# mabdullahsoyturk/Torch-Sputnik

Measured on AMD Instinct MI355X. Metric: SpMM effective GFLOP/s (2*nnz*N/t), M=N=K=4096 fp32, density 0.1, higher is better.
Workload: dtype f32

## Files before the change

torch_sputnik_amd/csrc/gen_spmm_flat.py:

```python
#!/usr/bin/env python3
import argparse

_ap = argparse.ArgumentParser()
_ap.add_argument("--mode", default="entry", choices=["entry", "group"])
_ap.add_argument("--layout", default="straight", choices=["straight", "diagonal"])
_ap.add_argument("out", nargs="?")
ARGS = _ap.parse_args()
GROUP = ARGS.mode == "group"

BK = 32
BK_SHIFT = 5
ROW_BYTES = 2048
ROW_SHIFT = 11
WIN_BYTES = 144
NSTRIP = 4
NPIECES = 4
ROWSTEP = 8

V_LANE, V_STAGE, V_PLAN, V_ROWS = "v0", "v1", "v2", "v3"
CUR_OFF, CUR_VAL = 4, 5
NXT_OFF, NXT_VAL, NXT_ROWS = 6, 7, 8
NN_OFF, NN_VAL, NN_ROWS = 10, 11, 12
PAIR = [16, 18, 20, 22]
VALT = [16, 18]
V_ADDR = 20
STRIP = [32, 40, 48, 56]
ACC = 64

S_STREAM, S_VALUES, S_CINFO, S_DENSE = "s[36:37]", "s[38:39]", "s[40:41]", "s[42:43]"
S_PITCH, S_KMAX, S_NCHUNKS, S_ROW0, S_LDS0, S_DEBUG = "s44", "s45", "s46", "s47", "s48", "s49"
S_REM, S_C, S_CIOFF, S_MINE, S_SB, S_NSW = "s50", "s51", "s56", "s57", "s76", "s77"
S_CI = ["s52", "s53", "s54", "s55"]
S_RET, S_BND = "s[58:59]", "s[60:61]"
S_ROWS = [62, 63, 64, 65]
S_IDX = [66, 67, 68, 69]
S_COLS = "s78"
S_T = ["s70", "s71", "s72", "s73", "s74", "s75"]

out = []


def emit(line):
    out.append(line)


def label(name):
    return f".L_{name}_%="


def strip_reads(ring, addr):
    s = STRIP[ring]
    emit(f"ds_read_b128 v[{s}:{s + 3}], v{addr}")
    emit(f"ds_read_b128 v[{s + 4}:{s + 7}], v{addr} offset:1024")


def fmas(src_pair, op_sel, ring):
    s = STRIP[ring]
    for q in range(4):
        emit(f"v_pk_fma_f32 v[{ACC + 2 * q}:{ACC + 2 * q + 1}], v[{src_pair}:{src_pair + 1}], "
             f"v[{s + 2 * q}:{s + 2 * q + 1}], v[{ACC + 2 * q}:{ACC + 2 * q + 1}] {op_sel}")


def entry_fma_stage(ring, lgkm):
    emit(f"s_waitcnt lgkmcnt({lgkm})")
    emit(f"s_set_gpr_idx_on s{S_IDX[ring]}, 0xc")
    fmas(PAIR[ring], "op_sel:[1,0,0] op_sel_hi:[1,1,1]", ring)
    emit("s_set_gpr_idx_off")


def entry_slot(slot):
    ring = slot % NSTRIP
    p = PAIR[ring]
    emit(f"{label(f'E_{slot}')}:")
    emit(f"s_sub_u32 {S_REM}, {S_REM}, 1")
    emit(f"s_cbranch_scc1 {label(f'bnd_{slot}')}")
    emit(f"v_mov_b64_dpp v[{p}:{p + 1}], v[{CUR_OFF}:{CUR_VAL}] row_newbcast:{slot} row_mask:0xf bank_mask:0xf")
    emit(f"s_bfe_u32 s{S_IDX[ring]}, s{S_ROWS[slot // 4]}, {hex(8 * (slot % 4) | (7 << 16))}")
    emit(f"v_add_u32 v{p}, v{p}, {V_LANE}")
    strip_reads(ring, p)
    entry_fma_stage((ring + 1) % NSTRIP, 2 * (NSTRIP - 1))


def group_entry_body(ring, slot):
    t = VALT[slot % 2]
    emit(f"v_mov_b32_dpp v{t}, v{CUR_VAL} row_newbcast:{slot} row_mask:0xf bank_mask:0xf")
    emit(f"s_bfe_u32 s{S_IDX[0]}, s{S_ROWS[slot // 4]}, {hex(8 * (slot % 4) | (7 << 16))}")
    emit(f"s_set_gpr_idx_on s{S_IDX[0]}, 0xc")
    fmas(t, "op_sel:[0,0,0] op_sel_hi:[0,1,1]", ring)
    emit("s_set_gpr_idx_off")


def group_start(ring, slot):
    emit(f"{label(f'N_{ring}_{slot}')}:")
    emit(f"s_sub_u32 {S_REM}, {S_REM}, 1")
    emit(f"s_cbranch_scc1 {label(f'bnd_{slot}')}")
    emit(f"v_mov_b32_dpp v{V_ADDR}, v{CUR_OFF} row_newbcast:{slot} row_mask:0xf bank_mask:0xf")
    emit(f"v_add_u32 v{V_ADDR}, v{V_ADDR}, {V_LANE}")
    strip_reads(ring, V_ADDR)
    emit(f"s_waitcnt lgkmcnt({2 * (NSTRIP - 1)})")


def first_groups():
    for i in range(NSTRIP - 1):
        emit(f"s_bfe_u32 {S_T[0]}, {S_COLS}, {hex(8 * i | (8 << 16))}")
        emit(f"s_lshl_b32 {S_T[0]}, {S_T[0]}, {ROW_SHIFT}")
        emit(f"v_add_u32 v{V_ADDR}, {S_T[0]}, {V_LANE}")
        strip_reads(i, V_ADDR)


def stage_chunk(chunk_sgpr):
    t_row, t_lds, t_r, t_lo, t_hi = S_T[1], S_T[2], S_T[3], S_T[4], S_T[5]
    emit(f"s_lshl_b32 {t_row}, {chunk_sgpr}, {BK_SHIFT}")
    emit(f"s_add_u32 {t_row}, {t_row}, {S_ROW0}")
    emit(f"s_and_b32 {t_lds}, {chunk_sgpr}, 1")
    emit(f"s_lshl_b32 {t_lds}, {t_lds}, 16")
    emit(f"s_add_u32 {t_lds}, {t_lds}, {S_LDS0}")
    for i in range(NPIECES):
        emit(f"s_add_u32 {t_r}, {t_row}, {ROWSTEP * i}")
        emit(f"s_min_u32 {t_r}, {t_r}, {S_KMAX}")
        emit(f"s_mul_hi_u32 {t_hi}, {t_r}, {S_PITCH}")
        emit(f"s_mul_i32 {t_lo}, {t_r}, {S_PITCH}")
        emit(f"s_add_u32 {t_lo}, {t_lo}, s42")
        emit(f"s_addc_u32 {t_hi}, {t_hi}, s43")
        emit(f"s_add_u32 m0, {t_lds}, {hex(ROWSTEP * i * ROW_BYTES)}")
        emit("s_nop 0")
        emit(f"global_load_lds_dwordx4 {V_STAGE}, s[{t_lo[1:]}:{t_hi[1:]}]")


def plan_load(off, rows):
    emit(f"global_load_dwordx2 v[{off}:{off + 1}], {V_PLAN}, {S_STREAM}")
    emit(f"global_load_dword v{rows}, {V_ROWS}, {S_STREAM}")
    emit(f"v_add_u32 {V_PLAN}, {hex(WIN_BYTES)}, {V_PLAN}")
    emit(f"v_add_u32 {V_ROWS}, {hex(WIN_BYTES)}, {V_ROWS}")


def gather(val):
    emit(f"global_load_dword v{val}, v{val}, {S_VALUES}")


def switch_window(tag):
    emit(f"s_cmp_lg_u32 {S_SB}, 0")
    emit(f"s_cbranch_scc1 {label('swc_' + tag)}")
    emit("s_waitcnt vmcnt(0)")
    emit(f"s_branch {label('swd_' + tag)}")
    emit(f"{label('swc_' + tag)}:")
    emit(f"s_waitcnt vmcnt({NPIECES})")
    emit(f"{label('swd_' + tag)}:")
    emit(f"s_mov_b32 {S_SB}, 0")
    emit(f"s_add_u32 {S_NSW}, {S_NSW}, 1")
    for i in range(4):
        emit(f"v_readlane_b32 s{S_ROWS[i]}, v{NXT_ROWS}, {i}")
    emit(f"v_bfe_u32 v{CUR_OFF}, v{NXT_OFF}, {8 if GROUP else 0}, 8")
    emit(f"v_mov_b32 v{CUR_VAL}, v{NXT_VAL}")
    emit(f"v_lshlrev_b32 v{CUR_OFF}, {ROW_SHIFT}, v{CUR_OFF}")
    emit(f"v_mov_b64 v[{NXT_OFF}:{NXT_VAL}], v[{NN_OFF}:{NN_VAL}]")
    emit(f"v_mov_b32 v{NXT_ROWS}, v{NN_ROWS}")
    emit(f"s_bitcmp1_b32 {S_DEBUG}, 3")
    emit(f"s_cbranch_scc1 {label('swskip_' + tag)}")
    gather(NXT_VAL)
    plan_load(NN_OFF, NN_ROWS)
    emit(f"{label('swskip_' + tag)}:")
    emit("s_nop 1")


def take_chunk_info():
    emit(f"s_mov_b32 {S_REM}, {S_CI[0] if GROUP else S_CI[3]}")
    if GROUP:
        emit(f"s_mov_b32 {S_COLS}, {S_CI[1]}")


def generate():
    emit("; ---- prologue ----")
    for r in list(range(ACC, ACC + 64)) + list(range(STRIP[0], STRIP[0] + 32)) + list(range(16, 24)):
        emit(f"v_mov_b32 v{r}, 0")
    for r in S_IDX:
        emit(f"s_mov_b32 s{r}, 0")
    emit(f"s_getpc_b64 {S_BND}")
    emit(f"{label('pc')}:")
    emit(f"s_add_u32 s60, s60, {label('boundary')}-{label('pc')}")
    emit("s_addc_u32 s61, s61, 0")
    plan_load(NXT_OFF, NXT_ROWS)
    plan_load(NN_OFF, NN_ROWS)
    emit("s_waitcnt vmcnt(2)")
    gather(NXT_VAL)
    emit(f"s_mov_b32 {S_T[0]}, 0")
    stage_chunk(S_T[0])
    emit(f"s_load_dwordx4 s[52:55], {S_CINFO}, 0x0")
    emit("s_waitcnt vmcnt(0) lgkmcnt(0)")
    emit("s_barrier")
    take_chunk_info()
    emit(f"s_load_dwordx4 s[52:55], {S_CINFO}, 0x10")
    emit(f"s_mov_b32 {S_CIOFF}, 32")
    emit(f"s_mov_b32 {S_C}, 0")
    emit(f"s_mov_b32 {S_NSW}, 0")
    emit(f"s_mov_b32 {S_SB}, 0")
    emit(f"s_mov_b32 {S_MINE}, 0")
    if GROUP:
        first_groups()
    emit(f"s_cmp_lt_u32 {S_NCHUNKS}, 2")
    emit(f"s_cbranch_scc1 {label('pro_nostage')}")
    emit(f"s_mov_b32 {S_T[0]}, 1")
    stage_chunk(S_T[0])
    emit(f"s_mov_b32 {S_SB}, 1")
    emit(f"s_mov_b32 {S_MINE}, 1")
    emit(f"{label('pro_nostage')}:")
    switch_window("pro")

    emit("; ---- main loop ----")
    if not GROUP:
        for slot in range(16):
            entry_slot(slot)
        switch_window("w")
        emit(f"s_branch {label('E_0')}")
    elif ARGS.layout == "straight":
        emit(f"s_branch {label(f'E_{NSTRIP - 1}_0')}")
        for ring in range(NSTRIP):
            for slot in range(16):
                emit(f"{label(f'E_{ring}_{slot}')}:")
                emit(f"s_bitcmp1_b32 s{S_ROWS[slot // 4]}, {8 * (slot % 4) + 7}")
                emit(f"s_cbranch_scc1 {label(f'N_{ring}_{slot}')}")
                emit(f"{label(f'B_{ring}_{slot}')}:")
                group_entry_body(ring, slot)
            switch_window(f"r{ring}")
            emit(f"s_branch {label(f'E_{ring}_0')}")
        emit("; ---- first entry of a column group ----")
        for ring in range(NSTRIP):
            for slot in range(16):
                group_start(ring, slot)
                emit(f"s_branch {label(f'B_{(ring + 1) % NSTRIP}_{slot}')}")
    else:
        emit(f"s_branch {label(f'E_{NSTRIP - 1}_0')}")
        for diag in range(NSTRIP):
            for slot in range(16):
                ring = (diag + slot) % NSTRIP
                emit(f"{label(f'E_{ring}_{slot}')}:")
                emit(f"s_bitcmp1_b32 s{S_ROWS[slot // 4]}, {8 * (slot % 4) + 7}")
                emit(f"s_cbranch_scc0 {label(f'B_{ring}_{slot}')}")
                group_start(ring, slot)
                emit(f"{label(f'B_{(ring + 1) % NSTRIP}_{slot}')}:")
                group_entry_body((ring + 1) % NSTRIP, slot)
            ring = (diag + 16) % NSTRIP
            switch_window(f"r{diag}")
            emit(f"s_branch {label(f'E_{ring}_0')}")

    emit("; ---- boundary stubs ----")
    for slot in range(16):
        emit(f"{label(f'bnd_{slot}')}:")
        emit(f"s_swappc_b64 {S_RET}, {S_BND}")
        if GROUP:
            emit(f"s_cbranch_scc1 {label('end')}")
            emit(f"s_branch {label(f'N_{NSTRIP - 1}_{slot}')}")
        else:
            emit(f"s_cbranch_scc1 {label(f'drain_{slot % NSTRIP}')}")
            emit(f"s_branch {label(f'E_{slot}')}")

    emit("; ---- boundary subroutine ----")
    emit(f"{label('boundary')}:")
    emit(f"s_bitcmp1_b32 {S_DEBUG}, 2")
    emit(f"s_cbranch_scc1 {label('bnodrain')}")
    emit("s_waitcnt lgkmcnt(0)")
    emit(f"{label('bnodrain')}:")
    emit(f"s_cmp_eq_u32 {S_MINE}, 0")
    emit(f"s_cbranch_scc1 {label('bvd')}")
    emit(f"s_bitcmp1_b32 {S_DEBUG}, 5")
    emit(f"s_cbranch_scc1 {label('bvd')}")
    for n in range(3):
        emit(f"s_cmp_eq_u32 {S_NSW}, {n}")
        emit(f"s_cbranch_scc1 {label(f'bv{n}')}")
    emit("s_waitcnt vmcnt(9)")
    emit(f"s_branch {label('bvd')}")
    for n in range(3):
        emit(f"{label(f'bv{n}')}:")
        emit(f"s_waitcnt vmcnt({3 * n})")
        if n < 2:
            emit(f"s_branch {label('bvd')}")
    emit(f"{label('bvd')}:")
    emit(f"s_bitcmp1_b32 {S_DEBUG}, 1")
    emit(f"s_cbranch_scc1 {label('bnobar')}")
    emit("s_barrier")
    emit(f"{label('bnobar')}:")
    emit(f"s_add_u32 {S_C}, {S_C}, 1")
    emit(f"s_cmp_eq_u32 {S_C}, {S_NCHUNKS}")
    emit(f"s_cbranch_scc1 {label('bret')}")
    take_chunk_info()
    emit(f"s_load_dwordx4 s[52:55], {S_CINFO}, {S_CIOFF}")
    emit(f"s_add_u32 {S_CIOFF}, {S_CIOFF}, 16")
    if GROUP:
        first_groups()
    emit(f"s_mov_b32 {S_NSW}, 0")
    emit(f"s_mov_b32 {S_MINE}, 0")
    emit(f"s_add_u32 {S_T[0]}, {S_C}, 1")
    emit(f"s_cmp_ge_u32 {S_T[0]}, {S_NCHUNKS}")
    emit(f"s_cbranch_scc1 {label('bnostage')}")
    emit(f"s_bitcmp1_b32 {S_DEBUG}, 0")
    emit(f"s_cbranch_scc1 {label('bnostage')}")
    stage_chunk(S_T[0])
    emit(f"s_add_u32 {S_SB}, {S_SB}, 1")
    emit(f"s_mov_b32 {S_MINE}, 1")
    emit(f"{label('bnostage')}:")
    emit(f"s_cmp_eq_u32 {S_C}, {S_NCHUNKS}")
    emit(f"{label('bret')}:")
    emit(f"s_setpc_b64 {S_RET}")

    if not GROUP:
        emit("; ---- drain: the three entries still in the pipeline ----")
        for ring in range(NSTRIP):
            emit(f"{label(f'drain_{ring}')}:")
            for j in range(1, NSTRIP):
                entry_fma_stage((ring + j) % NSTRIP, 2 * (NSTRIP - 1 - j))
            if ring < NSTRIP - 1:
                emit(f"s_branch {label('end')}")
    emit(f"{label('end')}:")
    emit("s_waitcnt vmcnt(0) lgkmcnt(0)")


def main():
    generate()
    text = "// GENERATED by gen_spmm_flat.py -- do not edit.\n" + "".join(
        f'"{line}\\n"\n' for line in out)
    if ARGS.out:
        with open(ARGS.out, "w") as f:
            f.write(text)
    else:
        print(text, end="")


if __name__ == "__main__":
    main()
```

torch_sputnik_amd/csrc/spmm_flat.hip:

```cpp
#include <algorithm>

#include "options.h"
#include "spmm_tiled_common.h"

namespace sputnik_hip {

namespace {

using namespace tiled;

constexpr int kBN = 512;
constexpr int kBK = 32;
constexpr int kWaves = 16;
constexpr int kRPW = 8;
constexpr int kBM = kWaves * kRPW;
constexpr int kAhead = 3;
constexpr int kDealPer = 256;
constexpr int kWindow = 16;
constexpr int kWindowBytes = 144;
constexpr int kTailWindows = 4;
constexpr int kMaxColumns = 65536;
constexpr unsigned kNewGroup = 0x80;


struct ChunkInfo {
  int groups;
  unsigned first_rows;
  unsigned unused;
  int entries;
};

__host__ __device__ inline size_t fill_tables_bytes(int nchunks) {
  return (sizeof(int) * (static_cast<size_t>(nchunks) * (kBK / 4 + 4) + 2 * kRPW + 2) + 15) / 16 * 16;
}
__device__ __forceinline__ int wave_sum(int v) {
#pragma unroll
  for (int o = 32; o > 0; o >>= 1) v += __shfl_xor(v, o);
  return v;
}
__device__ __forceinline__ int wave_inclusive_scan(int v, int lane) {
#pragma unroll
  for (int o = 1; o < 64; o <<= 1) {
    const int t = __shfl_up(v, o);
    if (lane >= o) v += t;
  }
  return v;
}

__global__ __launch_bounds__(kRPW * 64) void spmm_flat_fill_kernel(
    int m, int k, int slots, int nchunks, const int* __restrict__ row_indices,
    const int* __restrict__ row_offsets, const int* __restrict__ column_indices,
    int* __restrict__ row_ok, ChunkInfo* __restrict__ cinfo, int* __restrict__ gwin,
    unsigned char* __restrict__ stream, int stage_windows, int debug) {
  extern __shared__ unsigned lds[];
  constexpr int RPW = kRPW, BK = kBK, NT = RPW * 64;
  constexpr int WPC = BK / 4;
  constexpr int UN = 4;
  const int g = blockIdx.x, tid = threadIdx.x, lane = tid % 64, wave = tid / 64;
  const int groups = gridDim.x;
  unsigned* maskw = lds;
  int* ebase = reinterpret_cast<int*>(lds + nchunks * WPC);
  unsigned* nzmask = reinterpret_cast<unsigned*>(ebase + nchunks);
  unsigned* wprefix = nzmask + nchunks;
  int* scratch = reinterpret_cast<int*>(wprefix + 2 * nchunks);
  unsigned char* sbuf = reinterpret_cast<unsigned char*>(lds) + fill_tables_bytes(nchunks);

  for (int i = tid; i < nchunks * WPC; i += NT) maskw[i] = 0;
  const int slot = g * RPW + wave;
  const int entry = dealt_index(slot, slots, kDealPer);
  int p0 = 0, p1 = 0;
  if (entry < m) {
    const int row = row_indices[entry];
    p0 = row_offsets[row];
    p1 = row_offsets[row + 1];
  }
  int before = 0;
  for (int gp = tid; gp < g; gp += NT) {
    int rows[RPW], len = 0;
    int2 bounds[RPW];
#pragma unroll
    for (int r = 0; r < RPW; ++r) {
      const int e = dealt_index(gp * RPW + r, slots, kDealPer);
      rows[r] = e < m ? row_indices[e] : -1;
    }
#pragma unroll
    for (int r = 0; r < RPW; ++r) {
      typedef int int2_a4 __attribute__((ext_vector_type(2), aligned(4)));
      if (rows[r] >= 0) {
        const int2_a4 pair = *reinterpret_cast<const int2_a4*>(row_offsets + rows[r]);
        bounds[r] = make_int2(pair.x, pair.y);
      } else {
        bounds[r] = make_int2(0, 0);
      }
    }
#pragma unroll
    for (int r = 0; r < RPW; ++r) len += bounds[r].y - bounds[r].x;
    before += (len + kWindow - 1) / kWindow;
  }
  before = wave_sum(before);
  if (lane == 0) {
    scratch[wave] = before;
    scratch[RPW + wave] = p1 - p0;
  }
  if (tid == 0) scratch[2 * RPW] = 1;
  __syncthreads();
  int wbase = 0, total = 0;
#pragma unroll
  for (int r = 0; r < RPW; ++r) {
    wbase += scratch[r];
    total += scratch[RPW + r];
  }
  if (tid == 0) gwin[g] = wbase;
  unsigned char* my_stream = stream + static_cast<int64_t>(wbase) * kWindowBytes;
  const int windows = (total + kWindow - 1) / kWindow;

  bool ok = true;
  for (int base = p0; base < p1; base += 64 * UN) {
    int cur[UN], prev[UN];
#pragma unroll
    for (int u = 0; u < UN; ++u) {
      const int p = base + u * 64 + lane;
      cur[u] = p < p1 ? column_indices[p] : -2;
    }
    const int before_base = base > p0 ? column_indices[base - 1] : -1;
#pragma unroll
    for (int u = 0; u < UN; ++u) {
      const int up = __shfl_up(cur[u], 1);
      const int carry = u == 0 ? before_base : __shfl(cur[u == 0 ? 0 : u - 1], 63);
      prev[u] = lane == 0 ? carry : up;
    }
#pragma unroll
    for (int u = 0; u < UN; ++u) {
      if (cur[u] == -2) continue;
      if (cur[u] <= prev[u] || cur[u] >= k) ok = false;
      else atomicOr(&maskw[cur[u] >> 2], (1u << wave) << (8 * (cur[u] & 3)));
    }
  }
  const bool wave_ok = __builtin_amdgcn_ballot_w64(!ok) == 0;
  if (lane == 0) {
    row_ok[slot] = wave_ok ? 1 : 0;
    if (!wave_ok) scratch[2 * RPW] = 0;
  }
  __syncthreads();
  ChunkInfo* my_info = cinfo + static_cast<int64_t>(g) * (nchunks + 1);
  if (scratch[2 * RPW] == 0) {
    unsigned* w = reinterpret_cast<unsigned*>(my_stream);
    const int nwin = windows + (g == groups - 1 ? kTailWindows : 0);
    for (int i = tid; i < nwin * (kWindowBytes / 4); i += NT)
      w[i] = i % (kWindowBytes / 4) >= 32 ? 0x80808080u : 0u;
    for (int c = tid; c <= nchunks; c += NT) my_info[c] = ChunkInfo{0, 0u, 0u, 0};
    return;
  }

  if (debug & 0x100) return;
  for (int t0 = 0; t0 < nchunks * WPC; t0 += NT) {
    const int t = t0 + tid;
    const bool live = t < nchunks * WPC;
    const int c = t / WPC, i = t % WPC;
    const unsigned w = live ? maskw[t] : 0u;
    const int cnt = __popc(w);
    unsigned nz = 0u;
#pragma unroll
    for (int b = 0; b < 4; ++b)
      if ((w >> (8 * b)) & 0xffu) nz |= 1u << (4 * i + b);
    int incl = cnt;
#pragma unroll
    for (int o = 1; o < WPC; o <<= 1) {
      const int up = __shfl_up(incl, o, WPC);
      if (i >= o) incl += up;
    }
#pragma unroll
    for (int o = 1; o < WPC; o <<= 1) nz |= static_cast<unsigned>(__shfl_xor(static_cast<int>(nz), o, WPC));
    const int entries = __shfl(incl, WPC - 1, WPC);
    if (live) {
      reinterpret_cast<unsigned char*>(wprefix)[t] = static_cast<unsigned char>(incl - cnt);
      if (i == 0) {
        unsigned first = 0u, rest = nz;
        const int cgroups = __popc(nz);
#pragma unroll
        for (int q = 0; q < kAhead; ++q)
          if (rest) {
            first |= static_cast<unsigned>((c & 1) * BK + __ffs(rest) - 1) << (8 * q);
            rest &= rest - 1u;
          }
        ebase[c] = entries;
        nzmask[c] = nz;
        my_info[c] = ChunkInfo{cgroups, first, 0u, entries};
      }
    }
  }
  if (tid == 0) my_info[nchunks] = ChunkInfo{0, 0u, 0u, 0};
  __syncthreads();
  if (wave == 0) {
    int carry = 0;
    for (int c0 = 0; c0 < nchunks; c0 += 64) {
      const int c = c0 + lane;
      const int e = c < nchunks ? ebase[c] : 0;
      const int incl = wave_inclusive_scan(e, lane);
      if (c < nchunks) ebase[c] = carry + incl - e;
      carry += __shfl(incl, 63);
    }
  }
  __syncthreads();

  if (debug & 0x200) return;
  static_assert(WPC == 8, "two prefix words per chunk");
  const int nwin_out = windows + (g == groups - 1 ? kTailWindows : 0);
  const bool staged = nwin_out <= stage_windows && !(debug & 0x1000);
  unsigned char* const dst_stream = staged ? sbuf : my_stream;
  for (int base = p0; base < p1; base += 64 * UN) {
    int cols[UN];
#pragma unroll
    for (int u = 0; u < UN; ++u) {
      const int p = base + u * 64 + lane;
      cols[u] = p < p1 ? column_indices[p] : -1;
    }
#pragma unroll
    for (int u = 0; u < UN; ++u) {
      if (cols[u] < 0) continue;
      const int p = base + u * 64 + lane;
      const int col = cols[u], c = col / BK, j = col % BK;
      const unsigned w = maskw[c * WPC + j / 4];
      const int prefix = static_cast<int>((wprefix[2 * c + j / 16] >> (8 * ((j / 4) % 4))) & 0xffu) +
                         __popc(w & ((1u << (8 * (j & 3))) - 1u));
      const unsigned byte = (w >> (8 * (j & 3))) & 0xffu;
      const int own = __popc(byte & ((1u << wave) - 1u));
      const int pos = ebase[c] + prefix + own;
      unsigned rowbyte = wave * 8, tile_rows = static_cast<unsigned>((c & 1) * BK + j);
      if (own == 0) {
        rowbyte |= kNewGroup;
        unsigned ahead = j == BK - 1 ? 0u : nzmask[c] >> (j + 1);
        ahead &= ahead - 1u;
        ahead &= ahead - 1u;
        if (ahead) tile_rows |= static_cast<unsigned>((c & 1) * BK + j + __ffs(ahead)) << 8;
      }
      if (debug & 0x400) continue;
      unsigned char* block = dst_stream + static_cast<int64_t>(pos / kWindow) * kWindowBytes;
      const int e = pos % kWindow;
      *reinterpret_cast<uint2*>(block + 8 * e) = make_uint2(tile_rows, static_cast<unsigned>(p) * 4u);
      block[128 + e] = static_cast<unsigned char>(rowbyte);
    }
  }
  for (int pos = total + tid; pos < windows * kWindow; pos += NT) {
    unsigned char* block = dst_stream + static_cast<int64_t>(pos / kWindow) * kWindowBytes;
    *reinterpret_cast<uint2*>(block + 8 * (pos % kWindow)) = make_uint2(0u, 0u);
    block[128 + pos % kWindow] = static_cast<unsigned char>(kNewGroup);
  }
  if (g == groups - 1) {
    unsigned* w = reinterpret_cast<unsigned*>(dst_stream + static_cast<int64_t>(windows) * kWindowBytes);
    for (int i = tid; i < kTailWindows * (kWindowBytes / 4); i += NT)
      w[i] = i % (kWindowBytes / 4) >= 32 ? 0x80808080u : 0u;
  }
  if (staged) {
    __syncthreads();
    const uint4* src = reinterpret_cast<const uint4*>(sbuf);
    uint4* dst = reinterpret_cast<uint4*>(my_stream);
    for (int i = tid; i < nwin_out * (kWindowBytes / 16); i += NT) dst[i] = src[i];
  }
}

using v8f = float __attribute__((ext_vector_type(8)));

#define SPUTNIK_HIP_FLAT_ASM_OPERANDS                                                              \
      : "={v[64:71]}"(a0), "={v[72:79]}"(a1), "={v[80:87]}"(a2), "={v[88:95]}"(a3),                \
        "={v[96:103]}"(a4), "={v[104:111]}"(a5), "={v[112:119]}"(a6), "={v[120:127]}"(a7)          \
      : "{v0}"(lane_base), "{v1}"(stage_off), "{v2}"(plan_off), "{v3}"(rows_off),                  \
        "{s[36:37]}"(my_stream), "{s[38:39]}"(values), "{s[40:41]}"(my_info), "{s[42:43]}"(dense), \
        "{s44}"(pitch), "{s45}"(kmax), "{s46}"(nchunks), "{s47}"(row0), "{s48}"(lds0),             \
        "{s49}"(debug)                                                                             \
      : "memory", "m0", "scc", "v4", "v5", "v6", "v7", "v8", "v9", "v10", "v11", "v12", "v13",     \
        "v14", "v15", "v16", "v17", "v18", "v19", "v20", "v21", "v22", "v23", "v32", "v33", "v34", \
        "v35", "v36", "v37", "v38", "v39", "v40", "v41", "v42", "v43", "v44", "v45", "v46", "v47", \
        "v48", "v49", "v50", "v51", "v52", "v53", "v54", "v55", "v56", "v57", "v58", "v59", "v60", \
        "v61", "v62", "v63", "s50", "s51", "s52", "s53", "s54", "s55", "s56", "s57", "s58", "s59", \
        "s60", "s61", "s62", "s63", "s64", "s65", "s66", "s67", "s68", "s69", "s70", "s71", "s72", \
        "s73", "s74", "s75", "s76", "s77", "s78", "s79", "s80"

template <int LOOP>
__global__ __launch_bounds__(kWaves * 64) void spmm_flat_kernel(
    int m, int k, int n, int slots, int nchunks, int n_tiles, const int* __restrict__ row_indices,
    const float* __restrict__ values, int64_t values_stride, const ChunkInfo* __restrict__ cinfo,
    const int* __restrict__ gwin, const unsigned char* __restrict__ stream,
    const float* __restrict__ dense, int64_t dense_stride, float* __restrict__ out,
    int64_t out_stride, const int* __restrict__ row_ok, const int* __restrict__ row_offsets,
    const int* __restrict__ column_indices, int debug, Epilogue epi) {
  constexpr int RPW = kRPW, BM = kBM, BN = kBN, BK = kBK, VEC = 8;
  constexpr int PPR = VEC / 4;
  __shared__ float tile[2][BK * BN];

  const int lane = threadIdx.x % kWave;
  const int wave = __builtin_amdgcn_readfirstlane(threadIdx.x / kWave);

  const int bid = blockIdx.x;
  int ntile, mblock;
  int replica = blockIdx.y;
  const int xcd_cols = 1 << ((debug >> 13) & 3);
  if (xcd_cols > 1 && n_tiles == 8 && (gridDim.x / 8) % xcd_cols == 0) {
    const int xcd = bid % 8, i = bid / 8, col_groups = 8 / xcd_cols;
    ntile = (xcd % col_groups) * xcd_cols + i % xcd_cols;
    mblock = (xcd / col_groups) * ((gridDim.x / 8) / xcd_cols) + i / xcd_cols;
  } else if (n_tiles % 8 == 0) {
    const int per_xcd = n_tiles / 8;
    const int xcd = bid % 8, i = bid / 8;
    ntile = xcd * per_xcd + i % per_xcd;
    mblock = i / per_xcd;
  } else {
    const int work = xcd_local_index32();
    const int mblocks = gridDim.x / n_tiles;
    mblock = work % mblocks;
    ntile = (work / mblocks) % n_tiles;
    replica = work / (mblocks * n_tiles);
  }
  values += replica * values_stride;
  dense += replica * dense_stride;
  out += replica * out_stride;

  const int n0 = ntile * BN;
  const int slot0 = mblock * BM + wave * RPW;

  if (!block_rows_ok_wave(row_ok, mblock * BM, BM)) {
    for (int r = 0; r < RPW; ++r) {
      const int entry = dealt_index(slot0 + r, slots, kDealPer);
      if (entry >= m) continue;
      const int row = row_indices[entry];
#pragma unroll
      for (int h = 0; h < PPR; ++h) {
        if (n0 + h * 256 + lane * 4 >= n) continue;
        const int col = min(n0 + h * 256 + lane * 4, n - 4);
        const float4 acc4 = gather_row_strip(values, column_indices, row_offsets[row],
                                             row_offsets[row + 1], dense + col, n);
        *reinterpret_cast<float4*>(out + static_cast<int64_t>(row) * n + col) =
            apply_epilogue(acc4, epi, row);
      }
    }
    return;
  }

  const int group = slot0 / RPW;
  const unsigned char* my_stream =
      stream + static_cast<int64_t>(__builtin_amdgcn_readfirstlane(gwin[group])) * kWindowBytes;
  const ChunkInfo* my_info = cinfo + static_cast<int64_t>(group) * (nchunks + 1);
  const unsigned tile_lds = static_cast<unsigned>(reinterpret_cast<uintptr_t>(AS_LDS(&tile[0][0])));
  const unsigned lane_base = tile_lds + lane * 16;
  const unsigned stage_off =
      static_cast<unsigned>(min(n0 + (wave % PPR) * 256 + lane * 4, n - 4)) * 4u;
  const unsigned plan_off = (lane & 15) * 8, rows_off = 128 + (lane & 3) * 4;
  const int pitch = n * 4, kmax = k - 1, row0 = wave / PPR;
  const int lds0 = static_cast<int>(tile_lds) + (wave / PPR) * (BN * 4) + (wave % PPR) * 1024;

  v8f a0, a1, a2, a3, a4, a5, a6, a7;
  if constexpr (LOOP == 0) {
    asm volatile(
#include "spmm_flat_body_entry.inc"
        SPUTNIK_HIP_FLAT_ASM_OPERANDS);
  } else if constexpr (LOOP == 1) {
    asm volatile(
#include "spmm_flat_body_group_s.inc"
        SPUTNIK_HIP_FLAT_ASM_OPERANDS);
  } else {
    asm volatile(
#include "spmm_flat_body_group_d.inc"
        SPUTNIK_HIP_FLAT_ASM_OPERANDS);
  }

  const v8f acc[8] = {a0, a1, a2, a3, a4, a5, a6, a7};
#pragma unroll
  for (int r = 0; r < RPW; ++r) {
    const int entry = dealt_index(slot0 + r, slots, kDealPer);
    if (entry < m) {
      const int row = row_indices[entry];
#pragma unroll
      for (int h = 0; h < PPR; ++h)
        if (n0 + h * 256 + lane * 4 < n) {
          const int col = min(n0 + h * 256 + lane * 4, n - 4);
          const int f = r * VEC + 4 * h;
          *reinterpret_cast<float4*>(out + static_cast<int64_t>(row) * n + col) =
              apply_epilogue(make_float4(acc[f / 8][f % 8], acc[f / 8][f % 8 + 1],
                                         acc[f / 8][f % 8 + 2], acc[f / 8][f % 8 + 3]),
                             epi, row);
        }
    }
  }
}

struct FlatPlan {
  int slots, nchunks, n_tiles, groups;
  size_t row_ok_off, cinfo_off, gwin_off, stream_off, bytes;
};

FlatPlan make_flat_plan(int m, int k, int n, int nonzeros) {
  FlatPlan p;
  p.slots = ceil_div(m, kDealPer) * kDealPer;
  p.nchunks = ceil_div(k, kBK);
  p.n_tiles = ceil_div(n, kBN);
  p.groups = p.slots / kRPW;
  auto up = [](size_t v) { return (v + 255) / 256 * 256; };
  p.row_ok_off = 0;
  p.cinfo_off = row_ok_bytes(p.slots);
  p.gwin_off = up(p.cinfo_off + sizeof(ChunkInfo) * static_cast<size_t>(p.nchunks + 1) * p.groups);
  p.stream_off = up(p.gwin_off + sizeof(int) * static_cast<size_t>(p.groups));
  const size_t windows = static_cast<size_t>(nonzeros) / kWindow + p.groups + kTailWindows;
  p.bytes = up(p.stream_off + windows * kWindowBytes);
  return p;
}

int fill_stage_windows(int nchunks, int nonzeros, int groups) {
  const size_t tables = fill_tables_bytes(nchunks);
  if (tables + kWindowBytes > 64 * 1024) return 0;
  const int64_t room = static_cast<int64_t>((64 * 1024 - tables) / kWindowBytes);
  const int64_t want = (static_cast<int64_t>(nonzeros) / kWindow / groups) * 5 / 4 + kTailWindows + 2;
  return static_cast<int>(std::min(room, want));
}
size_t fill_lds_bytes(int nchunks, int stage_windows) {
  return fill_tables_bytes(nchunks) + static_cast<size_t>(stage_windows) * kWindowBytes;
}

int flat_mode(int m, int k, int nonzeros) {
  const int forced = options().spmm_sparse;
  if (forced >= 2 && forced <= 4) return forced - 2;
  const double d = static_cast<double>(nonzeros) / (static_cast<double>(m) * k);
  return d < 0.12 ? 0 : d < 0.36 ? 2 : 1;
}

}

static bool fill_lds_available(int k) {
  static const bool extended = [] {
    return hipFuncSetAttribute(reinterpret_cast<const void*>(spmm_flat_fill_kernel),
                               hipFuncAttributeMaxDynamicSharedMemorySize,
                               static_cast<int>(fill_lds_bytes(kMaxColumns / kBK, 0))) == hipSuccess;
  }();
  return extended || fill_lds_bytes(ceil_div(k, kBK), 0) <= 64 * 1024;
}

bool spmm_flat_applicable(int m, int k, int n, int nonzeros) {
  if (n < 4 || k < kBK || m < 64 || nonzeros < 16 * static_cast<int64_t>(m) ||
      nonzeros >= (1 << 29))
    return false;
  if (static_cast<int64_t>(ceil_div(n, kBN)) * kBN * 3 > static_cast<int64_t>(n) * 4) return false;
  return k <= kMaxColumns && m <= 16384 && fill_lds_available(k);
}

const char* spmm_flat_kernel_name(int m, int k, int nonzeros) {
  static const char* const names[] = {"spmm_flat_kernel<0>", "spmm_flat_kernel<1>", "spmm_flat_kernel<2>"};
  return names[flat_mode(m, k, nonzeros)];
}

int64_t spmm_flat_tiles(int m, int n) {
  return static_cast<int64_t>(ceil_div(m, kBM)) * ceil_div(n, kBN);
}

size_t spmm_flat_workspace_bytes(int m, int k, int n, int nonzeros) {
  return make_flat_plan(m, k, n, nonzeros).bytes;
}

int spmm_flat_plan(int m, int k, int n, int nonzeros, const int* row_indices,
                   const int* row_offsets, const int* column_indices, void* workspace,
                   hipStream_t stream) {
  const FlatPlan p = make_flat_plan(m, k, n, nonzeros);
  char* base = static_cast<char*>(workspace);
  if (!fill_lds_available(k)) return SPUTNIK_HIP_UNSUPPORTED;
  const int stage_windows = fill_stage_windows(p.nchunks, nonzeros, p.groups);
  hipLaunchKernelGGL(spmm_flat_fill_kernel, dim3(p.groups), dim3(kRPW * 64),
                     fill_lds_bytes(p.nchunks, stage_windows), stream, m, k, p.slots, p.nchunks, row_indices,
                     row_offsets, column_indices, reinterpret_cast<int*>(base + p.row_ok_off),
                     reinterpret_cast<ChunkInfo*>(base + p.cinfo_off),
                     reinterpret_cast<int*>(base + p.gwin_off),
                     reinterpret_cast<unsigned char*>(base + p.stream_off), stage_windows,
                     options().spmm_debug);
  return launch_status();
}

int xcd_columns_code(int k, int n, int nonzeros, int row_blocks) {
  const int forced = options().spmm_debug;
  if (forced & 0x8000) return (forced >> 13) & 3;
  if (ceil_div(n, kBN) != 8) return 0;
  const double stream = 13.0 * nonzeros, b = 4.0 * k * n;
  int best = 0;
  double best_bytes = stream * 8 + b;
  for (int code = 1; code <= 3; ++code) {
    const int c = 1 << code;
    if (row_blocks % c != 0) break;
    const double bytes = stream * 8 / c + b * c;
    if (bytes < 0.97 * best_bytes) {
      best = code;
      best_bytes = bytes;
    }
  }
  return best;
}

int spmm_flat_exec(int m, int k, int n, int nonzeros, int replicas, const int* row_indices,
                   const float* values, int64_t values_stride, const int* row_offsets,
                   const int* column_indices, const float* dense, int64_t dense_stride, float* out,
                   int64_t out_stride, const void* workspace, hipStream_t stream, Epilogue epi) {
  const FlatPlan p = make_flat_plan(m, k, n, nonzeros);
  const char* base = static_cast<const char*>(workspace);
#define SPUTNIK_HIP_LAUNCH_FLAT(LOOP)                                                              \
  hipLaunchKernelGGL((spmm_flat_kernel<LOOP>), dim3((p.slots / kBM) * p.n_tiles, replicas),        \
                     dim3(kWaves * 64), 0, stream, m, k, n, p.slots, p.nchunks, p.n_tiles,         \
                     row_indices, values, values_stride,                                           \
                     reinterpret_cast<const ChunkInfo*>(base + p.cinfo_off),                       \
                     reinterpret_cast<const int*>(base + p.gwin_off),                              \
                     reinterpret_cast<const unsigned char*>(base + p.stream_off), dense,           \
                     dense_stride, out, out_stride,                                                \
                     reinterpret_cast<const int*>(base + p.row_ok_off), row_offsets,               \
                     column_indices, debug_word, epi)
  const int debug_word = (options().spmm_debug & ~0xe000) |
                         (xcd_columns_code(k, n, nonzeros, p.slots / kBM) << 13);
  switch (flat_mode(m, k, nonzeros)) {
    case 0: SPUTNIK_HIP_LAUNCH_FLAT(0); break;
    case 1: SPUTNIK_HIP_LAUNCH_FLAT(1); break;
    default: SPUTNIK_HIP_LAUNCH_FLAT(2); break;
  }
#undef SPUTNIK_HIP_LAUNCH_FLAT
  return launch_status();
}

}
```

Before: 42040.

## Broadcast window values via LDS in group loop and route density 0.1 to it

In the group-mode inner loop, each window's 16 gathered values are written once to a per-wave LDS slot and read back as four b128 loads into registers. The FMAs then use op_sel to pick a value directly, which drops the per-entry DPP broadcast move. The address broadcast plus add is fused into a single v_add_u32_dpp. The density threshold for the entry loop drops from 0.12 to 0.09, so density 0.1 now runs the diagonal group loop; this costs extra LDS traffic and a waitcnt at each window switch.

```diff
diff --git a/torch_sputnik_amd/csrc/gen_spmm_flat.py b/torch_sputnik_amd/csrc/gen_spmm_flat.py
--- a/torch_sputnik_amd/csrc/gen_spmm_flat.py
+++ b/torch_sputnik_amd/csrc/gen_spmm_flat.py
@@ -22,8 +22,9 @@
 NXT_OFF, NXT_VAL, NXT_ROWS = 6, 7, 8
 NN_OFF, NN_VAL, NN_ROWS = 10, 11, 12
 PAIR = [16, 18, 20, 22]
-VALT = [16, 18]
-V_ADDR = 20
+V_ADDR = 9
+VALS = 16
+V_SLOT, V_SLOTW = "v13", "v14"
 STRIP = [32, 40, 48, 56]
 ACC = 64
 
@@ -82,11 +83,10 @@
 
 
 def group_entry_body(ring, slot):
-    t = VALT[slot % 2]
-    emit(f"v_mov_b32_dpp v{t}, v{CUR_VAL} row_newbcast:{slot} row_mask:0xf bank_mask:0xf")
+    h = slot & 1
     emit(f"s_bfe_u32 s{S_IDX[0]}, s{S_ROWS[slot // 4]}, {hex(8 * (slot % 4) | (7 << 16))}")
     emit(f"s_set_gpr_idx_on s{S_IDX[0]}, 0xc")
-    fmas(t, "op_sel:[0,0,0] op_sel_hi:[0,1,1]", ring)
+    fmas(VALS + (slot & ~1), f"op_sel:[{h},0,0] op_sel_hi:[{h},1,1]", ring)
     emit("s_set_gpr_idx_off")
 
 
@@ -94,8 +94,7 @@
     emit(f"{label(f'N_{ring}_{slot}')}:")
     emit(f"s_sub_u32 {S_REM}, {S_REM}, 1")
     emit(f"s_cbranch_scc1 {label(f'bnd_{slot}')}")
-    emit(f"v_mov_b32_dpp v{V_ADDR}, v{CUR_OFF} row_newbcast:{slot} row_mask:0xf bank_mask:0xf")
-    emit(f"v_add_u32 v{V_ADDR}, v{V_ADDR}, {V_LANE}")
+    emit(f"v_add_u32_dpp v{V_ADDR}, v{CUR_OFF}, {V_LANE} row_newbcast:{slot} row_mask:0xf bank_mask:0xf")
     strip_reads(ring, V_ADDR)
     emit(f"s_waitcnt lgkmcnt({2 * (NSTRIP - 1)})")
 
@@ -148,10 +147,15 @@
     emit(f"{label('swd_' + tag)}:")
     emit(f"s_mov_b32 {S_SB}, 0")
     emit(f"s_add_u32 {S_NSW}, {S_NSW}, 1")
+    if GROUP:
+        emit(f"ds_write_b32 {V_SLOTW}, v{NXT_VAL}")
+        for q in range(4):
+            emit(f"ds_read_b128 v[{VALS + 4 * q}:{VALS + 4 * q + 3}], {V_SLOT} offset:{16 * q}")
     for i in range(4):
         emit(f"v_readlane_b32 s{S_ROWS[i]}, v{NXT_ROWS}, {i}")
     emit(f"v_bfe_u32 v{CUR_OFF}, v{NXT_OFF}, {8 if GROUP else 0}, 8")
-    emit(f"v_mov_b32 v{CUR_VAL}, v{NXT_VAL}")
+    if not GROUP:
+        emit(f"v_mov_b32 v{CUR_VAL}, v{NXT_VAL}")
     emit(f"v_lshlrev_b32 v{CUR_OFF}, {ROW_SHIFT}, v{CUR_OFF}")
     emit(f"v_mov_b64 v[{NXT_OFF}:{NXT_VAL}], v[{NN_OFF}:{NN_VAL}]")
     emit(f"v_mov_b32 v{NXT_ROWS}, v{NN_ROWS}")
@@ -160,6 +164,8 @@
     gather(NXT_VAL)
     plan_load(NN_OFF, NN_ROWS)
     emit(f"{label('swskip_' + tag)}:")
+    if GROUP:
+        emit("s_waitcnt lgkmcnt(0)")
     emit("s_nop 1")
 
 
@@ -171,7 +177,8 @@
 
 def generate():
     emit("; ---- prologue ----")
-    for r in list(range(ACC, ACC + 64)) + list(range(STRIP[0], STRIP[0] + 32)) + list(range(16, 24)):
+    for r in list(range(ACC, ACC + 64)) + list(range(STRIP[0], STRIP[0] + 32)) + (
+            list(range(VALS, VALS + 16)) + [V_ADDR] if GROUP else list(range(16, 24))):
         emit(f"v_mov_b32 v{r}, 0")
     for r in S_IDX:
         emit(f"s_mov_b32 s{r}, 0")
diff --git a/torch_sputnik_amd/csrc/spmm_flat.hip b/torch_sputnik_amd/csrc/spmm_flat.hip
--- a/torch_sputnik_amd/csrc/spmm_flat.hip
+++ b/torch_sputnik_amd/csrc/spmm_flat.hip
@@ -261,15 +261,18 @@
 
 using v8f = float __attribute__((ext_vector_type(8)));
 
-#define SPUTNIK_HIP_FLAT_ASM_OPERANDS                                                              \
+#define SPUTNIK_HIP_FLAT_CLOBBERS_ENTRY "v5"
+#define SPUTNIK_HIP_FLAT_CLOBBERS_GROUP "v9", "v24", "v25", "v26", "v27", "v28", "v29", "v30", "v31"
+#define SPUTNIK_HIP_FLAT_ASM_OPERANDS(MODE_CLOBBERS)                                               \
       : "={v[64:71]}"(a0), "={v[72:79]}"(a1), "={v[80:87]}"(a2), "={v[88:95]}"(a3),                \
         "={v[96:103]}"(a4), "={v[104:111]}"(a5), "={v[112:119]}"(a6), "={v[120:127]}"(a7)          \
       : "{v0}"(lane_base), "{v1}"(stage_off), "{v2}"(plan_off), "{v3}"(rows_off),                  \
+        "{v13}"(slot_lds), "{v14}"(slot_lane),                                                     \
         "{s[36:37]}"(my_stream), "{s[38:39]}"(values), "{s[40:41]}"(my_info), "{s[42:43]}"(dense), \
         "{s44}"(pitch), "{s45}"(kmax), "{s46}"(nchunks), "{s47}"(row0), "{s48}"(lds0),             \
         "{s49}"(debug)                                                                             \
-      : "memory", "m0", "scc", "v4", "v5", "v6", "v7", "v8", "v9", "v10", "v11", "v12", "v13",     \
-        "v14", "v15", "v16", "v17", "v18", "v19", "v20", "v21", "v22", "v23", "v32", "v33", "v34", \
+      : "memory", "m0", "scc", MODE_CLOBBERS, "v4", "v6", "v7", "v8", "v10", "v11", "v12", "v16",  \
+        "v17", "v18", "v19", "v20", "v21", "v22", "v23", "v32", "v33", "v34",                      \
         "v35", "v36", "v37", "v38", "v39", "v40", "v41", "v42", "v43", "v44", "v45", "v46", "v47", \
         "v48", "v49", "v50", "v51", "v52", "v53", "v54", "v55", "v56", "v57", "v58", "v59", "v60", \
         "v61", "v62", "v63", "s50", "s51", "s52", "s53", "s54", "s55", "s56", "s57", "s58", "s59", \
@@ -287,6 +290,7 @@
   constexpr int RPW = kRPW, BM = kBM, BN = kBN, BK = kBK, VEC = 8;
   constexpr int PPR = VEC / 4;
   __shared__ float tile[2][BK * BN];
+  __shared__ __attribute__((aligned(16))) float value_slot[kWaves][kWindow];
 
   const int lane = threadIdx.x % kWave;
   const int wave = __builtin_amdgcn_readfirstlane(threadIdx.x / kWave);
@@ -345,6 +349,9 @@
   const unsigned stage_off =
       static_cast<unsigned>(min(n0 + (wave % PPR) * 256 + lane * 4, n - 4)) * 4u;
   const unsigned plan_off = (lane & 15) * 8, rows_off = 128 + (lane & 3) * 4;
+  const unsigned slot_lds =
+      static_cast<unsigned>(reinterpret_cast<uintptr_t>(AS_LDS(&value_slot[wave][0])));
+  const unsigned slot_lane = slot_lds + (lane & 15) * 4;
   const int pitch = n * 4, kmax = k - 1, row0 = wave / PPR;
   const int lds0 = static_cast<int>(tile_lds) + (wave / PPR) * (BN * 4) + (wave % PPR) * 1024;
 
@@ -352,15 +359,15 @@
   if constexpr (LOOP == 0) {
     asm volatile(
 #include "spmm_flat_body_entry.inc"
-        SPUTNIK_HIP_FLAT_ASM_OPERANDS);
+        SPUTNIK_HIP_FLAT_ASM_OPERANDS(SPUTNIK_HIP_FLAT_CLOBBERS_ENTRY));
   } else if constexpr (LOOP == 1) {
     asm volatile(
 #include "spmm_flat_body_group_s.inc"
-        SPUTNIK_HIP_FLAT_ASM_OPERANDS);
+        SPUTNIK_HIP_FLAT_ASM_OPERANDS(SPUTNIK_HIP_FLAT_CLOBBERS_GROUP));
   } else {
     asm volatile(
 #include "spmm_flat_body_group_d.inc"
-        SPUTNIK_HIP_FLAT_ASM_OPERANDS);
+        SPUTNIK_HIP_FLAT_ASM_OPERANDS(SPUTNIK_HIP_FLAT_CLOBBERS_GROUP));
   }
 
   const v8f acc[8] = {a0, a1, a2, a3, a4, a5, a6, a7};
@@ -419,7 +426,7 @@
   const int forced = options().spmm_sparse;
   if (forced >= 2 && forced <= 4) return forced - 2;
   const double d = static_cast<double>(nonzeros) / (static_cast<double>(m) * k);
-  return d < 0.12 ? 0 : d < 0.36 ? 2 : 1;
+  return d < 0.09 ? 0 : d < 0.36 ? 2 : 1;
 }
 
 }
```

New measurement: 41160. -2.1%, worse.
